# ViliamVadocz/takzero

Hardware: AMD Instinct MI355X
Metric: mcts_simulations_per_s (higher is better)
Workload: dtype f16

## Files before the change

bindings/takzero-hip-sys/src/lib.rs:

```rust
#![allow(non_camel_case_types, clippy::too_many_arguments)]
use std::os::raw::{c_char, c_int, c_uint, c_void};

pub const TZ_MAX_N: c_int = 6;
pub const TZ_MAX_SQUARES: c_int = 36;
pub const TZ_MAX_ACTIONS: c_int = 512;
pub const TZ_MAX_ACTIONS_6: c_int = 1024;
pub const TZ_OK: c_int = 0;
pub const TZ_EINVAL: c_int = -1;
pub const TZ_EPARSE: c_int = -2;
pub const TZ_EDEVICE: c_int = -3;
pub const TZ_ENOMEM: c_int = -4;
pub const TZ_ECAPACITY: c_int = -5;
pub const TZ_ESTATE: c_int = -6;
pub const TZ_ENUMERIC: c_int = -7;
pub const TZ_EMPTY: c_int = 0;
pub const TZ_FLAT: c_int = 1;
pub const TZ_WALL: c_int = 2;
pub const TZ_CAP: c_int = 3;
pub const TZ_EVAL_VALUE: c_int = 0;
pub const TZ_EVAL_WIN: c_int = 1;
pub const TZ_EVAL_LOSS: c_int = 2;
pub const TZ_EVAL_DRAW: c_int = 3;
pub const TZ_TERMINAL_NONE: c_int = -1;
pub const TZ_TERMINAL_WIN: c_int = 0;
// ... 168 lines not shown
    pub fn tz_reanalyze_take_text(ra: *mut TzReanalyze, out: *mut c_char, cap: u64, size_out: *mut u64) -> c_int;
    pub fn tz_reanalyze_run(ra: *mut TzReanalyze, directory: *const c_char, iterations: c_int, min_positions: c_int, suffix: *const c_char, reload: Option<unsafe extern "C" fn(*mut c_void) -> c_int>, reload_user: *mut c_void, wait_limit_s: f64) -> c_int;
    pub fn tz_compete(white: *mut TzSearch, black: *mut TzSearch, games: *const TzState, white_beta: f32, black_beta: f32, seed: u64, sampled_actions: c_int, search_budget: c_int, max_moves: c_int, result_out: *mut i32) -> c_int;
    pub fn tz_puzzle_benchmark(search: *mut TzSearch, puzzles: *const TzState, solutions: *const u16, count: c_int, win: c_int, seed: u64, sampled_actions: c_int, search_budget: c_int, result_out: *mut i32) -> c_int;
    pub fn tz_format_targets(n: c_int, count: c_int, states: *const TzState, moves: *const u16, policy: *const f32, nmoves: *const i32, amax: c_int, value: *const f32, ube: *const f32, out: *mut c_char, cap: u64, written_out: *mut u64) -> c_int;
    pub fn tz_parse_targets(text: *const c_char, len: u64, n: c_int, half_komi: c_int, max_targets: c_int, amax: c_int, states: *mut TzState, moves: *mut u16, policy: *mut f32, nmoves: *mut i32, value: *mut f32, ube: *mut f32, count_out: *mut i32, consumed_out: *mut u64, skipped_out: *mut i32) -> c_int;
    pub fn tz_trainer_create(board_n: c_int, arch: c_int, device_id: c_int, blocks: c_int, batch: c_int, learning_rate: f32, out: *mut *mut TzTrainer) -> c_int;
    pub fn tz_trainer_destroy(t: *mut TzTrainer) -> c_int;
    pub fn tz_trainer_tensor_count(t: *mut TzTrainer) -> c_int;
    pub fn tz_trainer_tensor_info(t: *mut TzTrainer, i: c_int, name_out: *mut c_char, name_cap: c_int, count_out: *mut u64) -> c_int;
    pub fn tz_trainer_set_tensor(t: *mut TzTrainer, name: *const c_char, what: c_int, data: *const f32, count: u64) -> c_int;
    pub fn tz_trainer_get_tensor(t: *mut TzTrainer, name: *const c_char, what: c_int, out: *mut f32, count: u64) -> c_int;
    pub fn tz_trainer_step(t: *mut TzTrainer, states: *const TzState, target_policy: *const f32, mask: *const u8, target_value: *const f32, target_ube: *const f32, train_ube: c_int, apply_step: c_int, losses_out: *mut f32) -> c_int;
    pub fn tz_trainer_outputs(t: *mut TzTrainer, policy_out: *mut f32, value_out: *mut f32, ube_out: *mut f32) -> c_int;
    pub fn tz_trainer_activation(t: *mut TzTrainer, layer: c_int, out: *mut f32, out_cap: u64) -> c_int;
    pub fn tz_trainer_shape(t: *mut TzTrainer, board_n_out: *mut c_int, batch_out: *mut c_int, arch_out: *mut c_int) -> c_int;
    pub fn tz_trainer_load(t: *mut TzTrainer, path: *const c_char) -> c_int;
    pub fn tz_trainer_save(t: *mut TzTrainer, path: *const c_char) -> c_int;
    pub fn tz_trainer_load_weights_mem(t: *mut TzTrainer, data: *const c_void, bytes: usize) -> c_int;
    pub fn tz_trainer_get_extras(t: *mut TzTrainer, out: *mut c_void, cap: u64, bytes_out: *mut u64) -> c_int;
    pub fn tz_trainer_from_net(t: *mut TzTrainer, net: *mut TzNet) -> c_int;
    pub fn tz_trainer_to_net(t: *mut TzTrainer, net: *mut TzNet) -> c_int;
    pub fn tz_learn_create(trainer: *mut TzTrainer, half_komi: c_int, seed: u64, selfplay_forced_uses: c_int, reanalyze_forced_uses: c_int, out: *mut *mut TzLearn) -> c_int;
    pub fn tz_learn_destroy(l: *mut TzLearn) -> c_int;
    pub fn tz_learn_feed(l: *mut TzLearn, which: c_int, path: *const c_char, model_steps: c_int, added_out: *mut u64) -> c_int;
    pub fn tz_learn_add_lines(l: *mut TzLearn, which: c_int, text: *const c_char, len: u64, model_steps: c_int, added_out: *mut u64) -> c_int;
    pub fn tz_learn_buffer_len(l: *mut TzLearn, which: c_int, len_out: *mut u64) -> c_int;
    pub fn tz_learn_step(l: *mut TzLearn, using_reanalyze: c_int, train_ube: c_int, augment: c_int, losses_out: *mut f32) -> c_int;
    pub fn tz_learn_last_batch(l: *mut TzLearn, states_out: *mut TzState, policy_out: *mut f32, mask_out: *mut u8, value_out: *mut f32, ube_out: *mut f32) -> c_int;
    pub fn tz_learn_run(l: *mut TzLearn, directory: *const c_char, starting_steps: i64, steps: i64, min_selfplay: c_int, min_reanalyze: c_int, steps_before_reanalyze: i64, read_interval_s: f64, sleep_s: f64, wait_limit_s: f64, on_step: Option<unsafe extern "C" fn(*mut c_void, i64, *const f32, *const TzState, c_int) -> c_int>, user: *mut c_void, model_steps_out: *mut i64) -> c_int;
    pub fn tz_learn_set_save_points(l: *mut TzLearn, steps_per_save: c_int, steps_per_checkpoint: c_int, hash_net: *mut TzNet) -> c_int;
    pub fn tz_device_math(op: c_int, a: *const f32, b: *const f32, out: *mut f32, n: c_int) -> c_int;
    pub fn tz_debug_conv_bench(net: *mut TzNet, variant: c_int, positions: c_int, iters: c_int, ms_out: *mut f32) -> c_int;
    pub fn tz_debug_tower_bench(net: *mut TzNet, variant: c_int, positions: c_int, iters: c_int, ms_out: *mut f32) -> c_int;
    pub fn tz_debug_net_clock(net: *mut TzNet, mhz_out: *mut f64, tower_us_out: *mut f64) -> c_int;
    pub fn tz_debug_net_stamps(net: *mut TzNet, out: *mut u64, max_groups: c_int, groups_out: *mut c_int) -> c_int;
}
```

include/takzero_hip.h:

```cpp
#ifndef TAKZERO_HIP_H
#define TAKZERO_HIP_H

#include <stddef.h>
#include <stdint.h>

#ifdef __cplusplus
extern "C" {
#endif

#define TZ_MAX_N 6
#define TZ_MAX_SQUARES 36
#define TZ_MAX_ACTIONS 512
#define TZ_MAX_ACTIONS_6 1024

#define TZ_OK 0
#define TZ_EINVAL (-1)
#define TZ_EPARSE (-2)
#define TZ_EDEVICE (-3)
#define TZ_ENOMEM (-4)
#define TZ_ECAPACITY (-5)
#define TZ_ESTATE (-6)
#define TZ_ENUMERIC (-7)

#define TZ_EMPTY 0
// ... 190 lines not shown
int tz_trainer_tensor_info(tz_trainer* t, int i, char* name_out, int name_cap, uint64_t* count_out);
int tz_trainer_set_tensor(tz_trainer* t, const char* name, int what, const float* data, uint64_t count);
int tz_trainer_get_tensor(tz_trainer* t, const char* name, int what, float* out, uint64_t count);
int tz_trainer_step(tz_trainer* t, const tz_state* states, const float* target_policy, const uint8_t* mask,
                    const float* target_value, const float* target_ube, int train_ube, int apply_step,
                    float* losses_out);
int tz_trainer_outputs(tz_trainer* t, float* policy_out, float* value_out, float* ube_out);
int tz_trainer_activation(tz_trainer* t, int layer, float* out, uint64_t out_cap);

int tz_trainer_shape(tz_trainer* t, int* board_n_out, int* batch_out, int* arch_out);
int tz_trainer_load(tz_trainer* t, const char* path);
int tz_trainer_save(tz_trainer* t, const char* path);
int tz_trainer_load_weights_mem(tz_trainer* t, const void* data, size_t bytes);
int tz_trainer_get_extras(tz_trainer* t, void* out, uint64_t cap, uint64_t* bytes_out);
int tz_trainer_from_net(tz_trainer* t, tz_net* net);
int tz_trainer_to_net(tz_trainer* t, tz_net* net);

typedef struct tz_learn tz_learn;
int tz_learn_create(tz_trainer* trainer, int half_komi, uint64_t seed, int selfplay_forced_uses, int reanalyze_forced_uses,
                    tz_learn** out);
int tz_learn_destroy(tz_learn* l);
int tz_learn_feed(tz_learn* l, int which, const char* path, int model_steps, uint64_t* added_out);
int tz_learn_add_lines(tz_learn* l, int which, const char* text, uint64_t len, int model_steps, uint64_t* added_out);
int tz_learn_buffer_len(tz_learn* l, int which, uint64_t* len_out);
int tz_learn_step(tz_learn* l, int using_reanalyze, int train_ube, int augment, float* losses_out);
int tz_learn_last_batch(tz_learn* l, tz_state* states_out, float* policy_out, uint8_t* mask_out, float* value_out, float* ube_out);
int tz_learn_run(tz_learn* l, const char* directory, int64_t starting_steps, int64_t steps, int min_selfplay, int min_reanalyze,
                 int64_t steps_before_reanalyze, double read_interval_s, double sleep_s, double wait_limit_s,
                 int (*on_step)(void*, int64_t, const float*, const tz_state*, int), void* user, int64_t* model_steps_out);
int tz_learn_set_save_points(tz_learn* l, int steps_per_save, int steps_per_checkpoint, tz_net* hash_net);

int tz_device_math(int op, const float* a, const float* b, float* out, int n);
int tz_debug_conv_bench(tz_net* net, int variant, int positions, int iters, float* ms_out);
int tz_debug_tower_bench(tz_net* net, int variant, int positions, int iters, float* ms_out);
int tz_debug_net_clock(tz_net* net, double* mhz_out, double* tower_us_out);
int tz_debug_net_stamps(tz_net* net, unsigned long long* out, int max_groups, int* groups_out);

#ifdef __cplusplus
}
#endif
#endif
```

takzero_amd/_lib.py:

```python
import ctypes as C
import os

import numpy as np

HERE = os.path.dirname(os.path.abspath(__file__))
LIB_PATH = os.path.join(HERE, "libtakzero_hip.so")
MAX_SQ = 36

STATE_DTYPE = np.dtype([
    ("colors", np.uint64, (MAX_SQ,)), ("height", np.uint8, (MAX_SQ,)), ("top", np.uint8, (MAX_SQ,)),
    ("stones", np.uint8, (2,)), ("caps", np.uint8, (2,)), ("to_move", np.uint8), ("n", np.uint8),
    ("half_komi", np.int8), ("pad0", np.uint8), ("ply", np.uint16), ("reversible_plies", np.uint16),
], align=True)
ROOT_INFO_DTYPE = np.dtype([
    ("visit_count", np.uint32), ("n_children", np.uint32), ("eval_tag", np.uint8),
    ("is_terminal_env", np.uint8), ("ply", np.uint16), ("eval_bits", np.uint32),
    ("std_dev", np.float32), ("logit", np.float32), ("probability", np.float32)], align=True)
assert STATE_DTYPE.itemsize == 376 and ROOT_INFO_DTYPE.itemsize == 28

SYMBOLS = [
    "tz_last_error", "tz_version", "tz_device_count", "tz_state_from_tps", "tz_state_to_tps", "tz_move_to_ptn",
    "tz_move_from_ptn", "tz_policy_size", "tz_input_channels", "tz_net_create", "tz_net_load_weights",
    "tz_net_load_weights_mem", "tz_net_destroy", "tz_net_eval", "tz_net_encode", "tz_net_forward_raw", "tz_net_hash_indices", "tz_net_load_bitset", "tz_net_save_bitset",
    "tz_search_create", "tz_search_destroy", "tz_search_set_positions", "tz_search_get_positions",
    "tz_search_new_openings", "tz_search_simulate", "tz_search_apply_noise", "tz_search_root_info",
    "tz_search_root_children", "tz_search_node", "tz_search_select_best_actions", "tz_search_improved_policy", "tz_search_ube_target",
    "tz_search_step", "tz_search_restart_terminal", "tz_search_gumbel_sh", "tz_search_counters", "tz_search_sync", "tz_search_pool_usage",
    "tz_search_profile", "tz_device_math", "tz_debug_conv_bench", "tz_debug_tower_bench", "tz_net_load_prepare", "tz_net_load_commit", "tz_net_load_discard", "tz_debug_net_clock", "tz_debug_net_stamps", "tz_search_terminal_details", "tz_search_play_moves",
    "tz_trainer_create", "tz_trainer_destroy", "tz_trainer_tensor_count", "tz_trainer_tensor_info",
    "tz_trainer_set_tensor", "tz_trainer_get_tensor", "tz_trainer_step", "tz_trainer_outputs", "tz_trainer_activation",
    "tz_format_targets", "tz_parse_targets", "tz_search_improved_policy_each", "tz_search_shape",
    "tz_selfplay_create", "tz_selfplay_destroy", "tz_selfplay_play_move", "tz_selfplay_counters", "tz_selfplay_take_text",
    "tz_selfplay_run", "tz_reanalyze_create", "tz_reanalyze_destroy", "tz_reanalyze_feed", "tz_reanalyze_iterate",
    "tz_reanalyze_take_text", "tz_reanalyze_run", "tz_compete", "tz_puzzle_benchmark", "tz_search_pool_overflows", "tz_trainer_shape",
    "tz_net_init_random", "tz_net_load_partial", "tz_net_save", "tz_net_clone", "tz_net_get_tensor", "tz_weights_convert", "tz_net_tensor_count", "tz_net_tensor_info",
    "tz_comm_unique_id", "tz_comm_rendezvous_id", "tz_comm_create_rccl", "tz_comm_create_fs", "tz_comm_destroy", "tz_comm_info",
    "tz_comm_all_gather", "tz_comm_take", "tz_comm_broadcast", "tz_comm_barrier", "tz_net_broadcast", "tz_selfplay_set_comm", "tz_selfplay_exchange",
    "tz_trainer_load", "tz_trainer_save", "tz_trainer_load_weights_mem", "tz_trainer_get_extras", "tz_trainer_from_net", "tz_trainer_to_net", "tz_learn_set_save_points",
    "tz_learn_create", "tz_learn_destroy", "tz_learn_feed", "tz_learn_add_lines", "tz_learn_buffer_len", "tz_learn_step", "tz_learn_run", "tz_learn_last_batch",
    "tz_search_simulate_batch", "tz_search_principal_variation", "tz_search_batch_profile",
    "tz_search_set_selection", "tz_search_get_selection",
]

_lib = None


class TakzeroError(RuntimeError):
    def __init__(self, code, msg):
        super().__init__("libtakzero_hip error %d: %s" % (code, msg))
        self.code = code


def load():
    global _lib
    if _lib is not None:
        return _lib
    if not os.path.exists(LIB_PATH):
        try:
            from . import build as _build

            _build.build()
# ... 48 lines not shown
    lib.tz_search_create.argtypes = [vp, ci, ci, ci, ci, ci, C.POINTER(vp)]
    lib.tz_search_destroy.argtypes = [vp]
    lib.tz_search_set_positions.argtypes = [vp, ci, vp, vp]
    lib.tz_search_get_positions.argtypes = [vp, vp]
    lib.tz_search_new_openings.argtypes = [vp, vp]
    lib.tz_search_simulate.argtypes = [vp, vp, ci]
    lib.tz_search_simulate_batch.argtypes = [vp, vp, ci, ci]
    lib.tz_search_batch_profile.argtypes = [vp] + [C.POINTER(C.c_double)] * 3 + [C.POINTER(C.c_uint64)]
    lib.tz_search_set_selection.argtypes = [vp, ci]
    lib.tz_search_get_selection.argtypes = [vp, C.POINTER(ci)]
    lib.tz_search_principal_variation.argtypes = [vp, ci, vp, ci, C.POINTER(ci)]
    lib.tz_search_apply_noise.argtypes = [vp, vp, ci, cf]
    lib.tz_search_root_info.argtypes = [vp, vp]
    lib.tz_search_root_children.argtypes = [vp, ci] + [vp] * 7
    lib.tz_search_node.argtypes = [vp, ci, vp, ci, vp, ci] + [vp] * 7
    lib.tz_search_select_best_actions.argtypes = [vp, vp]
    lib.tz_search_improved_policy.argtypes = [vp, cf, ci, vp]
    lib.tz_search_improved_policy_each.argtypes = [vp, vp, ci, vp]
    lib.tz_search_ube_target.argtypes = [vp, cf, vp]
    lib.tz_search_step.argtypes = [vp, vp]
    lib.tz_search_restart_terminal.argtypes = [vp, vp, vp]
    lib.tz_search_gumbel_sh.argtypes = [vp, vp, ci, ci, vp, ci, vp]
    lib.tz_search_counters.argtypes = [vp, C.POINTER(C.c_uint64), C.POINTER(C.c_uint64)]
    lib.tz_search_sync.argtypes = [vp]
    lib.tz_search_pool_overflows.argtypes = [vp, C.POINTER(C.c_uint64)]
    lib.tz_search_pool_usage.argtypes = [vp, C.POINTER(C.c_uint32), C.POINTER(C.c_uint32)]
    lib.tz_search_profile.argtypes = [vp, ci, C.POINTER(C.c_double), C.POINTER(C.c_uint64), C.POINTER(C.c_double),
                                      C.POINTER(C.c_uint64)]
    lib.tz_search_terminal_details.argtypes = [vp, vp, vp]
    lib.tz_search_play_moves.argtypes = [vp, vp, vp]
    lib.tz_device_math.argtypes = [ci, vp, vp, vp, ci]
    lib.tz_debug_conv_bench.argtypes = [vp, ci, ci, ci, C.POINTER(C.c_float)]
    lib.tz_debug_tower_bench.argtypes = [vp, ci, ci, ci, C.POINTER(C.c_float)]
    lib.tz_debug_net_clock.argtypes = [vp, C.POINTER(C.c_double), C.POINTER(C.c_double)]
    lib.tz_debug_net_stamps.argtypes = [vp, C.POINTER(C.c_uint64), C.c_int, C.POINTER(C.c_int)]
    lib.tz_net_load_prepare.argtypes = [vp, C.c_char_p, C.POINTER(vp)]
    lib.tz_net_load_commit.argtypes = [vp, vp]
    lib.tz_net_load_discard.argtypes = [vp]
    lib.tz_format_targets.argtypes = [ci, ci, vp, vp, vp, vp, ci, vp, vp, vp, C.c_uint64, C.POINTER(C.c_uint64)]
    lib.tz_parse_targets.argtypes = [vp, C.c_uint64, ci, ci, ci, ci, vp, vp, vp, vp, vp, vp, C.POINTER(C.c_int32),
                                     C.POINTER(C.c_uint64), C.POINTER(C.c_int32)]
    lib.tz_search_shape.argtypes = [vp] + [C.POINTER(ci)] * 4
    lib.tz_selfplay_create.argtypes = [vp, ci, C.c_uint64, ci, ci, ci, ci, C.POINTER(vp)]
    lib.tz_selfplay_destroy.argtypes = [vp]
    lib.tz_selfplay_play_move.argtypes = [vp]
    lib.tz_selfplay_counters.argtypes = [vp] + [C.POINTER(C.c_uint64)] * 3
    lib.tz_selfplay_take_text.argtypes = [vp, ci, vp, C.c_uint64, C.POINTER(C.c_uint64)]
    lib.tz_selfplay_run.argtypes = [vp, C.c_char_p, ci, ci, C.c_char_p, vp, vp, C.c_double]
    lib.tz_reanalyze_create.argtypes = [vp, ci, C.c_uint64, ci, ci, ci, ci, C.POINTER(vp)]
    lib.tz_reanalyze_destroy.argtypes = [vp]
    lib.tz_reanalyze_feed.argtypes = [vp, C.c_char_p, C.POINTER(C.c_uint64), C.POINTER(C.c_uint64)]
    lib.tz_reanalyze_iterate.argtypes = [vp]
    lib.tz_reanalyze_take_text.argtypes = [vp, vp, C.c_uint64, C.POINTER(C.c_uint64)]
    lib.tz_reanalyze_run.argtypes = [vp, C.c_char_p, ci, ci, C.c_char_p, vp, vp, C.c_double]
    lib.tz_compete.argtypes = [vp, vp, vp, cf, cf, C.c_uint64, ci, ci, ci, vp]
    lib.tz_puzzle_benchmark.argtypes = [vp, vp, vp, ci, ci, C.c_uint64, ci, ci, vp]
    lib.tz_trainer_shape.argtypes = [vp] + [C.POINTER(ci)] * 3
    lib.tz_learn_create.argtypes = [vp, ci, C.c_uint64, ci, ci, C.POINTER(vp)]
    lib.tz_learn_destroy.argtypes = [vp]
    lib.tz_learn_feed.argtypes = [vp, ci, C.c_char_p, ci, C.POINTER(C.c_uint64)]
    lib.tz_learn_add_lines.argtypes = [vp, ci, vp, C.c_uint64, ci, C.POINTER(C.c_uint64)]
    lib.tz_learn_buffer_len.argtypes = [vp, ci, C.POINTER(C.c_uint64)]
    lib.tz_learn_step.argtypes = [vp, ci, ci, ci, vp]
    lib.tz_learn_last_batch.argtypes = [vp, vp, vp, vp, vp, vp]
    lib.tz_learn_run.argtypes = [vp, C.c_char_p, C.c_int64, C.c_int64, ci, ci, C.c_int64, C.c_double, C.c_double, C.c_double, vp, vp,
                                 C.POINTER(C.c_int64)]
# ... 17 lines not shown
```

takzero_amd/csrc/tz_nn.hip:

```cpp
#include "tz_nn.h"
#include "tz_fp8.h"
#include "tz_fp6.h"
#include <type_traits>
#include "tz_ot.h"

#include <algorithm>
#include <cmath>
#include <cstdio>
#include <cstdlib>
#include <cstring>
#include <atomic>
#include <map>
#include <memory>
#include <mutex>
#include <thread>

int tz_nn_launch_split(int sp, int n, const void* net_args, int max_positions, hipStream_t st);
int tz_nn_launch_c6(int n, const void* net_args, int max_positions, hipStream_t st);
size_t tz_nn_c6_seed_bytes(int n, int max_positions);

namespace {

typedef float f32x4 __attribute__((ext_vector_type(4)));
typedef unsigned int u32x4 __attribute__((ext_vector_type(4)));
// ... 234 lines not shown
#pragma unroll
                for (int rt = 0; rt < RT; rt++) {
#pragma unroll
                    for (int j = 0; j < RN; j++)
                        acc[rt][j] = Elem<ET>::mfma(bq[kc & 3][j], av[rt], acc[rt][j]);
                    if constexpr ((ABL & 1) == 0) {
                        if (kc < 7) av[rt] = *reinterpret_cast<const ex8*>(lds + abase[rt] + (kc + 1 - (LAYOUT == 1 && kc >= 4 ? 4 : 0)) * KSTEP);
                        else av[rt] = *reinterpret_cast<const ex8*>(lds + abase[rt]);
                    }
                }
            }
        }
    } else {
        int yx[RT];
#pragma unroll
        for (int rt = 0; rt < RT; rt++) {
            const int r = rt * 16 + lr, px = r % NN;
            yx[rt] = r < ROWS ? ((px / NB) | ((px % NB) << 8)) : 0x7f7f;
        }
#pragma unroll
        for (int rt = 0; rt < RT; rt++)
#pragma unroll
            for (int j = 0; j < RN; j++) acc[rt][j] = f32x4{0.f, 0.f, 0.f, 0.f};
        const int nslices = (a.cin_pad + 255) / 256;
        constexpr int NLOAD = FROM_STATE ? 1 : (LROWS * 32 + NT - 1) / NT;
        uint4 stage[NLOAD];
        auto fetch_slice = [&](int slice) {
            const int cpr_s = min(256, a.cin_pad - slice * 256) / 8;
            const uint16_t* in = reinterpret_cast<const uint16_t*>(a.in) + (size_t)blockIdx.z * a.in_z + slice * 256;
#pragma unroll
            for (int i = 0; i < NLOAD; i++) {
                const int id = tid + i * NT, row = id >> 5, ci = id & 31;
                stage[i] = make_uint4(0, 0, 0, 0);
                if (row < valid_rows && ci < cpr_s) stage[i] = *reinterpret_cast<const uint4*>(in + (m0 + row) * a.in_stride + ci * 8);
            }
        };
        if constexpr (!FROM_STATE) fetch_slice(0);
        for (int slice = 0; slice < nslices; slice++) {
            const int cs = min(256, a.cin_pad - slice * 256);
            const int kcs = cs / 32, cpr = cs / 8;
            __syncthreads();
            if constexpr (FROM_STATE) {
                for (int row = tid; row < LROWS; row += NT) {
                    const bool ok = row < valid_rows;
                    const tz_state* s = nullptr;
                    int px = 0, fd = 0;
                    if (ok) {
                        const int pos = pos0 + row / NN;
                        px = row % NN;
                        s = a.states + (a.game_index ? a.game_index[pos] : pos);
                        fd = state_flat_diff<NB>(s);
                    }
                    for (int c8 = 0; c8 < cpr; c8++) {
                        ex8 v;
#pragma unroll
                        for (int k = 0; k < 8; k++) {
                            const int c = c8 * 8 + k;
                            v[k] = (ET)((ok && c < a.cin_real) ? plane_value<NB>(s, px, c, fd) : 0.0f);
                        }
                        *reinterpret_cast<ex8*>(lds + LdsImg<LAYOUT>::store_addr(row, c8, PLANE)) = v;
                    }
                }
            } else {
#pragma unroll
                for (int i = 0; i < NLOAD; i++) {
                    const int id = tid + i * NT, row = id >> 5, ci = id & 31;
                    if (row < LROWS && ci < cpr) *reinterpret_cast<uint4*>(lds + LdsImg<LAYOUT>::store_addr(row, ci, PLANE)) = stage[i];
                }
                if (slice + 1 < nslices) fetch_slice(slice + 1);
            }
            __syncthreads();
            ex8 bnext[RN];
#pragma unroll
            for (int j = 0; j < RN; j++) bnext[j] = wload(0, slice * 8, j);
            if constexpr (TAPS == 1) {
                int abase[RT];
                tap_bases<NB, RT, TAPS, LAYOUT>(yx, 0, lr, q, ZROW, abase);
                ex8 av[RT];
#pragma unroll
                for (int rt = 0; rt < RT; rt++) av[rt] = *reinterpret_cast<const ex8*>(lds + abase[rt]);
                for (int kc = 0; kc < kcs; kc++) {
                    ex8 bcur[RN];
#pragma unroll
                    for (int j = 0; j < RN; j++) bcur[j] = bnext[j];
                    if (kc + 1 < kcs) {
#pragma unroll
                        for (int j = 0; j < RN; j++) bnext[j] = wload(0, slice * 8 + kc + 1, j);
                    }
                    __builtin_amdgcn_sched_barrier(0);
#pragma unroll
                    for (int rt = 0; rt < RT; rt++) {
#pragma unroll
                        for (int j = 0; j < RN; j++) acc[rt][j] = Elem<ET>::mfma(bcur[j], av[rt], acc[rt][j]);
                        if (kc + 1 < kcs) av[rt] = *reinterpret_cast<const ex8*>(lds + abase[rt] + (kc + 1) * KSTEP);
                    }
                }
                continue;
            }
            for (int tap = 0; tap < TAPS; tap++) {
                int abase[RT];
                tap_bases<NB, RT, TAPS, LAYOUT>(yx, tap, lr, q, ZROW, abase);
                for (int kc = 0; kc < kcs; kc++) {
                    ex8 bcur[RN];
#pragma unroll
                    for (int j = 0; j < RN; j++) bcur[j] = bnext[j];
                    if (kc + 1 < kcs) {
#pragma unroll
                        for (int j = 0; j < RN; j++) bnext[j] = wload(tap, slice * 8 + kc + 1, j);
                    } else if (tap + 1 < TAPS) {
#pragma unroll
                        for (int j = 0; j < RN; j++) bnext[j] = wload(tap + 1, slice * 8, j);
                    }
#pragma unroll
                    for (int rt = 0; rt < RT; rt++) {
                        const ex8 av = *reinterpret_cast<const ex8*>(lds + abase[rt] + kc * KSTEP);
#pragma unroll
                        for (int j = 0; j < RN; j++)
                            acc[rt][j] = Elem<ET>::mfma(bcur[j], av, acc[rt][j]);
                    }
                }
            }
        }
    }

#pragma unroll
    for (int j = 0; j < RN; j++) {
        const int cbase = (ct0 + j) * 16 + q * 4;
        const f32x4 bias = *reinterpret_cast<const f32x4*>(a.bias + (size_t)blockIdx.z * a.bias_z + cbase);
#pragma unroll
        for (int rt = 0; rt < RT; rt++) {
            const int r = rt * 16 + lr;
            if (r >= valid_rows) continue;
            f32x4 v = acc[rt][j] + bias;
            const size_t o = (size_t)blockIdx.z * a.out_z + (m0 + r) * a.out_stride + cbase;
            if (a.has_res) {
                const ex4 rv = *reinterpret_cast<const ex4*>(reinterpret_cast<const uint16_t*>(a.residual) + o);
#pragma unroll
                for (int k = 0; k < 4; k++) v[k] += (float)rv[k];
            }
            if (a.relu) {
#pragma unroll
                for (int k = 0; k < 4; k++) v[k] = v[k] > 0.f ? v[k] : 0.f;
            }
            if (a.out_f32) {
                *reinterpret_cast<f32x4*>(reinterpret_cast<float*>(a.out) + o) = v;
            } else {
                ex4 ov;
#pragma unroll
                for (int k = 0; k < 4; k++) ov[k] = Elem<ET>::cvt(v[k]);
                *reinterpret_cast<ex4*>(reinterpret_cast<uint16_t*>(a.out) + o) = ov;
            }
        }
    }
}

struct TowerArgs {
    const uint16_t* in;
    uint16_t* out;
    const uint16_t* w;
    const float* bias;
    const int32_t* count_dev;
    int count_host;
    int nlayers;
};

template <int NB, int P, int OPT = 0, typename ET = __bf16>
__global__ __launch_bounds__(512, 2) void tower_mfma_kernel(TowerArgs a) {
    typedef typename Elem<ET>::x8 ex8;
    typedef typename Elem<ET>::x4 ex4;
    constexpr int RN = 2, TAPS = 9, LAYOUT = 1, NT = 512;
    constexpr int NN = NB * NB, ROWS = P * NN, RT = (ROWS + 15) / 16, LROWS = RT * 16 + 8, ZROW = RT * 16;
    constexpr int PLANE = LROWS * LDS_ROWB, KSTEP = PLANE;
// ... 2487 lines not shown
}

__host__ __device__ constexpr int ppt_small(int nb) { return nb == 1 ? 64 : nb == 3 ? 7 : nb == 4 ? 6 : nb == 5 ? 4 : 3; }

int conv_cfg() {
    static int cfg = -1;
    if (cfg < 0) {
        const char* e = getenv("TZ_CONV_CFG");
        cfg = e ? atoi(e) : 0;
    }
    return cfg;
}

template <int NB, int P, int NW, int RN, int TAPS, bool FROM_STATE, bool SINGLE, int ABL = 0, int LAYOUT = 1, typename ET = __bf16, int OCC = 2>
int launch_conv(const ConvArgs& a, int max_positions, int n_blocks_y, hipStream_t st) {
    constexpr int NN = NB * NB, RT = (P * NN + 15) / 16, LROWS = RT * 16 + 8;
    const size_t smem = LdsImg<LAYOUT>::bytes(LROWS);
    auto kern = conv_mfma_kernel<NB, P, RN, TAPS, FROM_STATE, ABL, SINGLE, NW, LAYOUT, ET, OCC>;
    static bool attr_done[64] = {};
    int attr_dev = 0;
    TZ_HIP(hipGetDevice(&attr_dev));
    bool& attr_set = attr_done[attr_dev & 63];
    if (!attr_set) {
        TZ_HIP(hipFuncSetAttribute(reinterpret_cast<const void*>(kern), hipFuncAttributeMaxDynamicSharedMemorySize, (int)smem));
        attr_set = true;
    }
    dim3 grid((max_positions + P - 1) / P, n_blocks_y, a.groups > 1 ? a.groups : 1);
    hipLaunchKernelGGL(kern, grid, dim3(NW * 64), smem, st, a);
    hipError_t e = hipGetLastError();
    if (e != hipSuccess) return tz_fail(TZ_EDEVICE, std::string("conv launch: ") + hipGetErrorString(e));
    return TZ_OK;
}

int linear_grouped_bf16(int precision, const uint16_t* w, const float* bias, int groups, int cin_pad, int cout_pad, const void* in,
                        int in_stride, int in_z, void* out, int out_stride, int out_z, bool relu, bool out_f32,
                        const int32_t* count_dev, int count_host, int max_positions, hipStream_t st) {
    ConvArgs a;
    memset(&a, 0, sizeof a);
    a.in = in;
    a.count_dev = count_dev;
    a.count_host = count_host;
    a.w = w;
    a.bias = bias;
    a.out = out;
    a.cin_pad = cin_pad;
    a.kc_total = cin_pad / 32;
    a.ct_total = cout_pad / 16;
    a.out_stride = out_stride;
    a.cin_real = cin_pad;
    a.relu = relu;
    a.out_f32 = out_f32;
    a.in_stride = in_stride;
    a.groups = groups;
    a.in_z = in_z;
    a.w_z_frags = a.kc_total * a.ct_total;
    a.bias_z = cout_pad;
    a.out_z = out_z;
    if (max_positions <= 128) {
        if (prec_is_f16(precision)) return launch_conv<1, 32, 8, 2, 1, false, false, 0, 1, _Float16>(a, max_positions, cout_pad / 256, st);
        return launch_conv<1, 32, 8, 2, 1, false, false>(a, max_positions, cout_pad / 256, st);
    }
    if (prec_is_f16(precision)) return launch_conv<1, 128, 8, 2, 1, false, false, 0, 1, _Float16>(a, max_positions, cout_pad / 256, st);
    return launch_conv<1, 128, 8, 2, 1, false, false>(a, max_positions, cout_pad / 256, st);
}

template <int NB, typename ET>
int conv_board(const ConvArgs& a, int cout_pad, bool from_state, int max_positions, hipStream_t st) {
    constexpr int PA = ppt_for(NB), PB = ppt_small(NB);
    const bool wide = cout_pad % 256 == 0;
    const int by = wide ? cout_pad / 256 : cout_pad / 128;
    if (conv_cfg() == 0) {
        if (from_state) return launch_conv<NB, PA, 8, 2, 9, true, false, 0, 1, ET>(a, max_positions, by, st);
        if (wide) return launch_conv<NB, PA, 8, 2, 9, false, true, 0, 1, ET>(a, max_positions, by, st);
        return launch_conv<NB, PA, 8, 1, 9, false, true, 0, 1, ET>(a, max_positions, by, st);
    }
    if (from_state) return launch_conv<NB, PB, 4, 4, 9, true, false, 0, 1, ET>(a, max_positions, by, st);
    if (wide) return launch_conv<NB, PB, 4, 4, 9, false, true, 0, 1, ET>(a, max_positions, by, st);
    return launch_conv<NB, PB, 4, 2, 9, false, true, 0, 1, ET>(a, max_positions, by, st);
}

template <typename ET>
int conv_dispatch(int n, bool board, const ConvArgs& a, int cout_pad, bool from_state, int max_positions, hipStream_t st) {
    if (!board) return launch_conv<1, 64, 8, 2, 1, false, false, 0, 1, ET>(a, max_positions, cout_pad / 256, st);
    switch (n) {
        case 3: return conv_board<3, ET>(a, cout_pad, from_state, max_positions, st);
        case 4: return conv_board<4, ET>(a, cout_pad, from_state, max_positions, st);
        case 5: return conv_board<5, ET>(a, cout_pad, from_state, max_positions, st);
        case 6: return conv_board<6, ET>(a, cout_pad, from_state, max_positions, st);
    }
    return tz_fail(TZ_EINVAL, "conv: unsupported board size");
}

int conv_bf16(tz_net* net, const ConvW& L, const void* in, const tz_state* states, const int32_t* gidx,
              const int32_t* count_dev, int count_host, int max_positions, const void* residual, void* out,
              int out_stride, bool relu, bool out_f32, bool board, hipStream_t st) {
    ConvArgs a;
// ... 1051 lines not shown
                case 0: rc = launch_conv<5, ppt_for(5), 8, 2, 9, false, true, 0>(a, positions, 1, net->stream); break;
#ifdef TZ_ABLATIONS
                case 1: rc = launch_conv<5, ppt_for(5), 8, 2, 9, false, true, 1>(a, positions, 1, net->stream); break;
                case 2: rc = launch_conv<5, ppt_for(5), 8, 2, 9, false, true, 2>(a, positions, 1, net->stream); break;
                case 3: rc = launch_conv<5, ppt_for(5), 8, 2, 9, false, true, 3>(a, positions, 1, net->stream); break;
                case 4: rc = launch_conv<5, ppt_for(5), 8, 2, 1, false, true, 0>(a, positions, 1, net->stream); break;
                case 20: rc = launch_conv<5, ppt_for(5), 8, 2, 9, false, true, 0, 0>(a, positions, 1, net->stream); break;
                case 21: rc = launch_conv<5, ppt_for(5), 8, 2, 9, false, true, 1, 0>(a, positions, 1, net->stream); break;
                case 23: rc = launch_conv<5, ppt_for(5), 8, 2, 9, false, true, 3, 0>(a, positions, 1, net->stream); break;
                case 30: rc = launch_conv<5, ppt_for(5), 4, 4, 9, false, true, 0, 1, __bf16, 1>(a, positions, 1, net->stream); break;
                case 31: rc = launch_conv<5, ppt_for(5), 4, 4, 9, false, true, 1, 1, __bf16, 1>(a, positions, 1, net->stream); break;
                case 33: rc = launch_conv<5, ppt_for(5), 4, 4, 9, false, true, 3, 1, __bf16, 1>(a, positions, 1, net->stream); break;
                case 10: rc = launch_conv<5, ppt_small(5), 4, 4, 9, false, true, 0>(a, positions, 1, net->stream); break;
                case 11: rc = launch_conv<5, ppt_small(5), 4, 4, 9, false, true, 1>(a, positions, 1, net->stream); break;
                case 12: rc = launch_conv<5, ppt_small(5), 4, 4, 9, false, true, 2>(a, positions, 1, net->stream); break;
                case 13: rc = launch_conv<5, ppt_small(5), 4, 4, 9, false, true, 3>(a, positions, 1, net->stream); break;
                case 14: rc = launch_conv<5, ppt_small(5), 4, 4, 1, false, true, 0>(a, positions, 1, net->stream); break;
#endif
                default: rc = tz_fail(TZ_EINVAL, "tz_debug_conv_bench: unknown variant (the ablation variants need a build with --ablations)");
            }
        }
        return rc;
    };
    if ((rc = run(3))) return rc;
    TZ_HIP(hipEventRecord(e0, net->stream));
    if ((rc = run(iters))) return rc;
    TZ_HIP(hipEventRecord(e1, net->stream));
    TZ_HIP(hipEventSynchronize(e1));
    float ms = 0.f;
    TZ_HIP(hipEventElapsedTime(&ms, e0, e1));
    (void)hipEventDestroy(e0);
    (void)hipEventDestroy(e1);
    *ms_out = ms / iters;
    return TZ_OK;
}

int tz_debug_tower_bench(tz_net* net, int variant, int positions, int iters, float* ms_out) {
    if (!net || !net->loaded || net->n != 5 || net->precision != TZ_PREC_BF16 || !net->tower_w)
        return tz_fail(TZ_EINVAL, "tz_debug_tower_bench: needs a loaded 5x5 bf16 network");
    TZ_HIP(hipSetDevice(net->device));
    int rc = tz_net_ensure_batch(net, positions);
    if (rc) return rc;
    {
        std::vector<uint16_t> h((size_t)positions * 25 * FILTERS);
        uint32_t x = 999u;
        for (auto& v : h) {
            x = x * 1664525u + 1013904223u;
            v = (x >> 31) ? 0 : f2bf((float)((x >> 8) % 10001) * 1e-4f);
        }
        TZ_HIP(hipMemcpy(net->act_a, h.data(), h.size() * 2, hipMemcpyHostToDevice));
    }
    TowerArgs a;
    a.in = reinterpret_cast<const uint16_t*>(net->act_a);
    a.out = reinterpret_cast<uint16_t*>(net->act_b);
    a.w = net->tower_w;
    a.bias = net->tower_bias;
    a.count_dev = nullptr;
    a.count_host = positions;
    a.nlayers = 2 * net->blocks;
    hipEvent_t e0, e1;
    TZ_HIP(hipEventCreate(&e0));
    TZ_HIP(hipEventCreate(&e1));
    auto run = [&](int n) -> int {
        int r = TZ_OK;
        for (int i = 0; i < n && !r; i++) {
            switch (variant) {
// ... 346 lines not shown
```

Baseline: 1.498 million.

## Add dedicated pipelined MFMA linear kernel for RND MLP layers with adaptive tile size

Adds a linear_mfma_kernel for the large-batch RND linear layers. It double-buffers 256-channel activation slices in LDS through buffer loads, prefetches weight fragments two k-steps ahead, and replaces the generic conv kernel for batches above 128 positions. The tile is 64 positions when the 128-position grid would leave CUs idle, otherwise 128. The aim is to hide global and LDS latency behind MFMA work and to fill the GPU better on small grids, at the cost of another kernel and more template instantiations. It also adds debug benchmark and buffer-readback entry points and ablation hooks in the conv kernel.

```diff
diff --git a/bindings/takzero-hip-sys/src/lib.rs b/bindings/takzero-hip-sys/src/lib.rs
--- a/bindings/takzero-hip-sys/src/lib.rs
+++ b/bindings/takzero-hip-sys/src/lib.rs
@@ -224,6 +224,8 @@
     pub fn tz_learn_set_save_points(l: *mut TzLearn, steps_per_save: c_int, steps_per_checkpoint: c_int, hash_net: *mut TzNet) -> c_int;
     pub fn tz_device_math(op: c_int, a: *const f32, b: *const f32, out: *mut f32, n: c_int) -> c_int;
     pub fn tz_debug_conv_bench(net: *mut TzNet, variant: c_int, positions: c_int, iters: c_int, ms_out: *mut f32) -> c_int;
+    pub fn tz_debug_linear_bench(net: *mut TzNet, variant: c_int, layer: c_int, positions: c_int, iters: c_int, ms_out: *mut f32) -> c_int;
+    pub fn tz_debug_rnd_buffer(net: *mut TzNet, which: c_int, out: *mut c_void, bytes: usize) -> c_int;
     pub fn tz_debug_tower_bench(net: *mut TzNet, variant: c_int, positions: c_int, iters: c_int, ms_out: *mut f32) -> c_int;
     pub fn tz_debug_net_clock(net: *mut TzNet, mhz_out: *mut f64, tower_us_out: *mut f64) -> c_int;
     pub fn tz_debug_net_stamps(net: *mut TzNet, out: *mut u64, max_groups: c_int, groups_out: *mut c_int) -> c_int;
diff --git a/include/takzero_hip.h b/include/takzero_hip.h
--- a/include/takzero_hip.h
+++ b/include/takzero_hip.h
@@ -246,6 +246,8 @@
 
 int tz_device_math(int op, const float* a, const float* b, float* out, int n);
 int tz_debug_conv_bench(tz_net* net, int variant, int positions, int iters, float* ms_out);
+int tz_debug_linear_bench(tz_net* net, int variant, int layer, int positions, int iters, float* ms_out);
+int tz_debug_rnd_buffer(tz_net* net, int which, void* out, size_t bytes);
 int tz_debug_tower_bench(tz_net* net, int variant, int positions, int iters, float* ms_out);
 int tz_debug_net_clock(tz_net* net, double* mhz_out, double* tower_us_out);
 int tz_debug_net_stamps(tz_net* net, unsigned long long* out, int max_groups, int* groups_out);
diff --git a/takzero_amd/_lib.py b/takzero_amd/_lib.py
--- a/takzero_amd/_lib.py
+++ b/takzero_amd/_lib.py
@@ -26,7 +26,7 @@
     "tz_search_new_openings", "tz_search_simulate", "tz_search_apply_noise", "tz_search_root_info",
     "tz_search_root_children", "tz_search_node", "tz_search_select_best_actions", "tz_search_improved_policy", "tz_search_ube_target",
     "tz_search_step", "tz_search_restart_terminal", "tz_search_gumbel_sh", "tz_search_counters", "tz_search_sync", "tz_search_pool_usage",
-    "tz_search_profile", "tz_device_math", "tz_debug_conv_bench", "tz_debug_tower_bench", "tz_net_load_prepare", "tz_net_load_commit", "tz_net_load_discard", "tz_debug_net_clock", "tz_debug_net_stamps", "tz_search_terminal_details", "tz_search_play_moves",
+    "tz_search_profile", "tz_device_math", "tz_debug_conv_bench", "tz_debug_tower_bench", "tz_debug_linear_bench", "tz_debug_rnd_buffer", "tz_net_load_prepare", "tz_net_load_commit", "tz_net_load_discard", "tz_debug_net_clock", "tz_debug_net_stamps", "tz_search_terminal_details", "tz_search_play_moves",
     "tz_trainer_create", "tz_trainer_destroy", "tz_trainer_tensor_count", "tz_trainer_tensor_info",
     "tz_trainer_set_tensor", "tz_trainer_get_tensor", "tz_trainer_step", "tz_trainer_outputs", "tz_trainer_activation",
     "tz_format_targets", "tz_parse_targets", "tz_search_improved_policy_each", "tz_search_shape",
@@ -141,6 +141,8 @@
     lib.tz_device_math.argtypes = [ci, vp, vp, vp, ci]
     lib.tz_debug_conv_bench.argtypes = [vp, ci, ci, ci, C.POINTER(C.c_float)]
     lib.tz_debug_tower_bench.argtypes = [vp, ci, ci, ci, C.POINTER(C.c_float)]
+    lib.tz_debug_linear_bench.argtypes = [vp, ci, ci, ci, ci, C.POINTER(C.c_float)]
+    lib.tz_debug_rnd_buffer.argtypes = [vp, ci, vp, C.c_size_t]
     lib.tz_debug_net_clock.argtypes = [vp, C.POINTER(C.c_double), C.POINTER(C.c_double)]
     lib.tz_debug_net_stamps.argtypes = [vp, C.POINTER(C.c_uint64), C.c_int, C.POINTER(C.c_int)]
     lib.tz_net_load_prepare.argtypes = [vp, C.c_char_p, C.POINTER(vp)]
diff --git a/takzero_amd/csrc/tz_nn.hip b/takzero_amd/csrc/tz_nn.hip
--- a/takzero_amd/csrc/tz_nn.hip
+++ b/takzero_amd/csrc/tz_nn.hip
@@ -290,6 +290,10 @@
             for (int i = 0; i < NLOAD; i++) {
                 const int id = tid + i * NT, row = id >> 5, ci = id & 31;
                 stage[i] = make_uint4(0, 0, 0, 0);
+                if constexpr ((ABL & 4) != 0) {
+                    stage[i] = make_uint4(0x38003c00u + row, 0x3a003400u, 0x3c003800u + ci, 0x34003a00u);
+                    continue;
+                }
                 if (row < valid_rows && ci < cpr_s) stage[i] = *reinterpret_cast<const uint4*>(in + (m0 + row) * a.in_stride + ci * 8);
             }
         };
@@ -319,7 +323,7 @@
                         *reinterpret_cast<ex8*>(lds + LdsImg<LAYOUT>::store_addr(row, c8, PLANE)) = v;
                     }
                 }
-            } else {
+            } else if ((ABL & 4) == 0 || slice == 0) {
 #pragma unroll
                 for (int i = 0; i < NLOAD; i++) {
                     const int id = tid + i * NT, row = id >> 5, ci = id & 31;
@@ -341,7 +345,7 @@
                     ex8 bcur[RN];
 #pragma unroll
                     for (int j = 0; j < RN; j++) bcur[j] = bnext[j];
-                    if (kc + 1 < kcs) {
+                    if ((ABL & 2) == 0 && kc + 1 < kcs) {
 #pragma unroll
                         for (int j = 0; j < RN; j++) bnext[j] = wload(0, slice * 8 + kc + 1, j);
                     }
@@ -350,7 +354,7 @@
                     for (int rt = 0; rt < RT; rt++) {
 #pragma unroll
                         for (int j = 0; j < RN; j++) acc[rt][j] = Elem<ET>::mfma(bcur[j], av[rt], acc[rt][j]);
-                        if (kc + 1 < kcs) av[rt] = *reinterpret_cast<const ex8*>(lds + abase[rt] + (kc + 1) * KSTEP);
+                        if ((ABL & 1) == 0 && kc + 1 < kcs) av[rt] = *reinterpret_cast<const ex8*>(lds + abase[rt] + (kc + 1) * KSTEP);
                     }
                 }
                 continue;
@@ -396,6 +400,151 @@
 #pragma unroll
                 for (int k = 0; k < 4; k++) v[k] += (float)rv[k];
             }
+            if (a.relu) {
+#pragma unroll
+                for (int k = 0; k < 4; k++) v[k] = v[k] > 0.f ? v[k] : 0.f;
+            }
+            if (a.out_f32) {
+                *reinterpret_cast<f32x4*>(reinterpret_cast<float*>(a.out) + o) = v;
+            } else {
+                ex4 ov;
+#pragma unroll
+                for (int k = 0; k < 4; k++) ov[k] = Elem<ET>::cvt(v[k]);
+                *reinterpret_cast<ex4*>(reinterpret_cast<uint16_t*>(a.out) + o) = ov;
+            }
+        }
+    }
+}
+
+template <int P, typename ET = __bf16, int ABL = 0>
+__global__ __launch_bounds__(512, 2) void linear_mfma_kernel(ConvArgs a) {
+    typedef typename Elem<ET>::x8 ex8;
+    typedef typename Elem<ET>::x4 ex4;
+    constexpr int NT = 512, NW = 8, RN = 2, RT = P / 16;
+    constexpr int PLANE = P * LDS_ROWB + 64, IMG = 8 * PLANE;
+    constexpr int NLOAD = P * 32 / NT;
+    static_assert(P % 16 == 0 && (P * 32) % NT == 0 && NLOAD <= 8, "a slice is stored within its 8 k-steps");
+    static_assert((RT - 1) * 16 * LDS_ROWB + 7 * PLANE < 65536, "fragment reads are one base register + immediates");
+    extern __shared__ __attribute__((aligned(16))) unsigned char lds[];
+    const int count = a.count_dev ? *a.count_dev : a.count_host;
+    const int pos0 = blockIdx.x * P;
+    if (pos0 >= count) return;
+    const int tid = threadIdx.x, lane = tid & 63;
+    const int wave = __builtin_amdgcn_readfirstlane(tid >> 6);
+    const int q = lane >> 4, lr = lane & 15;
+    const int valid_rows = min(P, count - pos0);
+    const size_t m0 = (size_t)pos0;
+    const int ct0 = (blockIdx.y * NW + wave) * RN;
+    const __amdgpu_buffer_rsrc_t wrsrc = __builtin_amdgcn_make_buffer_rsrc(
+        const_cast<uint16_t*>(a.w), 0, (a.groups > 1 ? a.groups * a.w_z_frags : a.kc_total * a.ct_total) * 1024, 0x00020000);
+    const int lane16 = lane * 16;
+    const int kc_total = a.kc_total;
+    auto wload = [&](int kcg, int j) -> ex8 {
+        const int frag = (int)blockIdx.z * a.w_z_frags + kcg * a.ct_total + (ct0 + j);
+        const u32x4 r = __builtin_amdgcn_raw_buffer_load_b128(wrsrc, lane16, frag * 1024, 0);
+        return __builtin_bit_cast(ex8, r);
+    };
+    const int nslices = (a.cin_pad + 255) / 256;
+    const int srow = tid >> 5, sci = tid & 31;
+    const int pitch = a.in_stride * 2;
+    const __amdgpu_buffer_rsrc_t arsrc = __builtin_amdgcn_make_buffer_rsrc(
+        const_cast<uint16_t*>(reinterpret_cast<const uint16_t*>(a.in) + (size_t)blockIdx.z * a.in_z + m0 * a.in_stride), 0,
+        (valid_rows - 1) * pitch + a.cin_pad * 2, 0x00020000);
+    const int voff0 = srow * pitch + sci * 16;
+    uint4 stage[NLOAD];
+    auto fetch_piece = [&](int slice_off, int i) {
+        if constexpr ((ABL & 4) == 0) {
+            const u32x4 r = __builtin_amdgcn_raw_buffer_load_b128(arsrc, voff0 + i * 16 * pitch + slice_off, 0, 0);
+            stage[i] = __builtin_bit_cast(uint4, r);
+        } else {
+            stage[i] = make_uint4(0x38003c00u + srow, 0x3a003400u, 0x3c003800u + sci, 0x34003a00u);
+        }
+    };
+    constexpr int NO_SLICE = 0x40000000;
+    const int sbase = LdsImg<1>::store_addr(srow, sci, PLANE);
+    const int abase = LdsImg<1>::read_base(true, lr, q, 0);
+
+#pragma unroll
+    for (int i = 0; i < NLOAD; i++) fetch_piece(0, i);
+    ex8 bq[4][RN];
+#pragma unroll
+    for (int j = 0; j < RN; j++) {
+        bq[0][j] = wload(0, j);
+        bq[1][j] = wload(min(1, kc_total - 1), j);
+    }
+    f32x4 acc[RT][RN];
+#pragma unroll
+    for (int rt = 0; rt < RT; rt++)
+#pragma unroll
+        for (int j = 0; j < RN; j++) acc[rt][j] = f32x4{0.f, 0.f, 0.f, 0.f};
+#pragma unroll
+    for (int i = 0; i < NLOAD; i++) *reinterpret_cast<uint4*>(lds + sbase + i * 16 * LDS_ROWB) = stage[i];
+    {
+        const int off = nslices > 1 ? 512 : NO_SLICE;
+#pragma unroll
+        for (int i = 0; i < NLOAD; i++) fetch_piece(off, i);
+    }
+    __syncthreads();
+
+    ex8 av[RT];
+    auto k_step = [&](auto store, int kc, int g, const unsigned char* img, unsigned char* other, int next2_off) {
+        constexpr bool STORE = decltype(store)::value;
+        if constexpr ((ABL & 2) == 0) {
+#pragma unroll
+            for (int j = 0; j < RN; j++) bq[(kc + 2) & 3][j] = wload(min(g + 2, kc_total - 1), j);
+        }
+        if constexpr (STORE && (ABL & 4) == 0) {
+            if (kc < NLOAD) {
+                *reinterpret_cast<uint4*>(other + kc * 16 * LDS_ROWB) = stage[kc];
+                fetch_piece(next2_off, kc);
+            }
+        }
+        __builtin_amdgcn_sched_barrier(0);
+#pragma unroll
+        for (int rt = 0; rt < RT; rt++) {
+#pragma unroll
+            for (int j = 0; j < RN; j++) acc[rt][j] = Elem<ET>::mfma(bq[kc & 3][j], av[rt], acc[rt][j]);
+            if constexpr ((ABL & 1) == 0) {
+                if (kc < 7) av[rt] = *reinterpret_cast<const ex8*>(img + rt * 16 * LDS_ROWB + (kc + 1) * PLANE);
+            }
+        }
+    };
+    int slice = 0;
+    for (; slice + 1 < nslices; slice++) {
+        const unsigned char* img = lds + (slice & 1) * IMG + abase;
+        unsigned char* other = lds + ((slice & 1) ^ 1) * IMG + sbase;
+        const int next2_off = slice + 2 < nslices ? (slice + 2) * 512 : NO_SLICE;
+#pragma unroll
+        for (int rt = 0; rt < RT; rt++) av[rt] = *reinterpret_cast<const ex8*>(img + rt * 16 * LDS_ROWB);
+#pragma unroll
+        for (int kc = 0; kc < 8; kc++) k_step(std::true_type{}, kc, slice * 8 + kc, img, other, next2_off);
+        __syncthreads();
+    }
+    {
+        const unsigned char* img = lds + (slice & 1) * IMG + abase;
+        const int kcs = kc_total - slice * 8;
+#pragma unroll
+        for (int rt = 0; rt < RT; rt++) av[rt] = *reinterpret_cast<const ex8*>(img + rt * 16 * LDS_ROWB);
+        if (kcs == 8) {
+#pragma unroll
+            for (int kc = 0; kc < 8; kc++) k_step(std::false_type{}, kc, slice * 8 + kc, img, nullptr, 0);
+        } else {
+#pragma unroll
+            for (int kc = 0; kc < 7; kc++)
+                if (kc < kcs) k_step(std::false_type{}, kc, slice * 8 + kc, img, nullptr, 0);
+        }
+    }
+
+#pragma unroll
+    for (int j = 0; j < RN; j++) {
+        const int cbase = (ct0 + j) * 16 + q * 4;
+        const f32x4 bias = *reinterpret_cast<const f32x4*>(a.bias + (size_t)blockIdx.z * a.bias_z + cbase);
+#pragma unroll
+        for (int rt = 0; rt < RT; rt++) {
+            const int r = rt * 16 + lr;
+            if (r >= valid_rows) continue;
+            f32x4 v = acc[rt][j] + bias;
+            const size_t o = (size_t)blockIdx.z * a.out_z + (m0 + r) * a.out_stride + cbase;
             if (a.relu) {
 #pragma unroll
                 for (int k = 0; k < 4; k++) v[k] = v[k] > 0.f ? v[k] : 0.f;
@@ -2949,6 +3098,43 @@
     return TZ_OK;
 }
 
+template <int P, typename ET, int ABL = 0>
+int launch_linear(const ConvArgs& a, int max_positions, int n_blocks_y, hipStream_t st) {
+    constexpr size_t smem = 2 * 8 * ((size_t)P * LDS_ROWB + 64);
+    auto kern = linear_mfma_kernel<P, ET, ABL>;
+    static bool attr_done[64] = {};
+    int attr_dev = 0;
+    TZ_HIP(hipGetDevice(&attr_dev));
+    bool& attr_set = attr_done[attr_dev & 63];
+    if (!attr_set) {
+        TZ_HIP(hipFuncSetAttribute(reinterpret_cast<const void*>(kern), hipFuncAttributeMaxDynamicSharedMemorySize, (int)smem));
+        attr_set = true;
+    }
+    dim3 grid((max_positions + P - 1) / P, n_blocks_y, a.groups > 1 ? a.groups : 1);
+    hipLaunchKernelGGL(kern, grid, dim3(512), smem, st, a);
+    hipError_t e = hipGetLastError();
+    if (e != hipSuccess) return tz_fail(TZ_EDEVICE, std::string("linear launch: ") + hipGetErrorString(e));
+    return TZ_OK;
+}
+
+int rnd_gemm_cfg() {
+    static int cfg = -1;
+    if (cfg < 0) {
+        const char* e = getenv("TZ_RND_GEMM");
+        cfg = !e ? 0 : !strcmp(e, "conv") ? 1 : !strcmp(e, "p128") ? 128 : !strcmp(e, "p64") ? 64 : 0;
+    }
+    return cfg;
+}
+
+int device_cu_count() {
+    static int cus[64] = {};
+    int dev = 0;
+    if (hipGetDevice(&dev) != hipSuccess) return 256;
+    int& c = cus[dev & 63];
+    if (c == 0 && hipDeviceGetAttribute(&c, hipDeviceAttributeMultiprocessorCount, dev) != hipSuccess) c = 256;
+    return c;
+}
+
 int linear_grouped_bf16(int precision, const uint16_t* w, const float* bias, int groups, int cin_pad, int cout_pad, const void* in,
                         int in_stride, int in_z, void* out, int out_stride, int out_z, bool relu, bool out_f32,
                         const int32_t* count_dev, int count_host, int max_positions, hipStream_t st) {
@@ -2977,8 +3163,18 @@
         if (prec_is_f16(precision)) return launch_conv<1, 32, 8, 2, 1, false, false, 0, 1, _Float16>(a, max_positions, cout_pad / 256, st);
         return launch_conv<1, 32, 8, 2, 1, false, false>(a, max_positions, cout_pad / 256, st);
     }
-    if (prec_is_f16(precision)) return launch_conv<1, 128, 8, 2, 1, false, false, 0, 1, _Float16>(a, max_positions, cout_pad / 256, st);
-    return launch_conv<1, 128, 8, 2, 1, false, false>(a, max_positions, cout_pad / 256, st);
+    const int cfg = rnd_gemm_cfg();
+    if (cfg == 1) {
+        if (prec_is_f16(precision)) return launch_conv<1, 128, 8, 2, 1, false, false, 0, 1, _Float16>(a, max_positions, cout_pad / 256, st);
+        return launch_conv<1, 128, 8, 2, 1, false, false>(a, max_positions, cout_pad / 256, st);
+    }
+    const bool half_tiles = cfg ? cfg == 64 : (max_positions + 127) / 128 * (cout_pad / 256) * groups < device_cu_count();
+    if (half_tiles) {
+        if (prec_is_f16(precision)) return launch_linear<64, _Float16>(a, max_positions, cout_pad / 256, st);
+        return launch_linear<64, __bf16>(a, max_positions, cout_pad / 256, st);
+    }
+    if (prec_is_f16(precision)) return launch_linear<128, _Float16>(a, max_positions, cout_pad / 256, st);
+    return launch_linear<128, __bf16>(a, max_positions, cout_pad / 256, st);
 }
 
 template <int NB, typename ET>
@@ -4096,6 +4292,102 @@
     (void)hipEventDestroy(e0);
     (void)hipEventDestroy(e1);
     *ms_out = ms / iters;
+    return TZ_OK;
+}
+
+int tz_debug_linear_bench(tz_net* net, int variant, int layer, int positions, int iters, float* ms_out) {
+    if (!net || !net->loaded || !net->has_rnd || net->n != 5 || net->precision == TZ_PREC_F32 || layer < 0 || layer > 2 || positions <= 128 || iters < 1)
+        return tz_fail(TZ_EINVAL, "tz_debug_linear_bench: needs a loaded 5x5 net5 in a 16-bit precision, layer 0..2 and more than 128 positions");
+    TZ_HIP(hipSetDevice(net->device));
+    int rc = tz_net_ensure_batch(net, positions);
+    if (rc) return rc;
+    const int in_pad = (net->cin * net->nn + 31) / 32 * 32;
+    const bool f16 = prec_is_f16(net->precision);
+    {
+        std::vector<uint16_t> h((size_t)positions * 2048);
+        uint32_t x = 4242u;
+        for (auto& v : h) {
+            x = x * 1664525u + 1013904223u;
+            const float f = ((int)(x >> 8) % 20001 - 10000) * 1e-4f;
+            v = f16 ? f2h(f) : f2bf(f);
+        }
+        TZ_HIP(hipMemcpy(net->rnd_in, h.data(), (size_t)positions * in_pad * 2, hipMemcpyHostToDevice));
+        TZ_HIP(hipMemcpy(net->rnd_h1, h.data(), h.size() * 2, hipMemcpyHostToDevice));
+        TZ_HIP(hipMemcpy(net->rnd_h2, h.data(), h.size() * 2, hipMemcpyHostToDevice));
+    }
+    ConvArgs a;
+    memset(&a, 0, sizeof a);
+    const int groups = layer == 0 ? 1 : 2, cin_pad = layer == 0 ? in_pad : 1024, cout_pad = layer == 0 ? 2048 : layer == 1 ? 1024 : 512;
+    a.in = layer == 0 ? net->rnd_in : layer == 1 ? net->rnd_h1 : net->rnd_h2;
+    a.out = layer == 0 ? net->rnd_h1 : layer == 1 ? net->rnd_h2 : (void*)net->rnd_out;
+    a.count_host = positions;
+    a.w = net->rndw[layer];
+    a.bias = net->rndb[layer];
+    a.cin_pad = a.cin_real = cin_pad;
+    a.kc_total = cin_pad / 32;
+    a.ct_total = cout_pad / 16;
+    a.out_stride = layer == 2 ? 1024 : 2048;
+    a.relu = layer != 2;
+    a.out_f32 = layer == 2;
+    a.in_stride = layer == 0 ? in_pad : 2048;
+    a.groups = groups;
+    a.in_z = layer == 0 ? 0 : 1024;
+    a.w_z_frags = a.kc_total * a.ct_total;
+    a.bias_z = cout_pad;
+    a.out_z = layer == 0 ? 0 : layer == 1 ? 1024 : 512;
+    const int by = cout_pad / 256;
+    auto one = [&](auto et) -> int {
+        typedef std::remove_pointer_t<decltype(et)> ET;
+        switch (variant) {
+            case 0: return launch_conv<1, 128, 8, 2, 1, false, false, 0, 1, ET>(a, positions, by, net->stream);
+            case 10: return launch_linear<128, ET>(a, positions, by, net->stream);
+            case 20: return launch_linear<64, ET>(a, positions, by, net->stream);
+#ifdef TZ_ABLATIONS
+            case 1: return launch_conv<1, 128, 8, 2, 1, false, false, 1, 1, ET>(a, positions, by, net->stream);
+            case 2: return launch_conv<1, 128, 8, 2, 1, false, false, 2, 1, ET>(a, positions, by, net->stream);
+            case 3: return launch_conv<1, 128, 8, 2, 1, false, false, 3, 1, ET>(a, positions, by, net->stream);
+            case 7: return launch_conv<1, 128, 8, 2, 1, false, false, 7, 1, ET>(a, positions, by, net->stream);
+            case 11: return launch_linear<128, ET, 1>(a, positions, by, net->stream);
+            case 12: return launch_linear<128, ET, 2>(a, positions, by, net->stream);
+            case 13: return launch_linear<128, ET, 3>(a, positions, by, net->stream);
+            case 17: return launch_linear<128, ET, 7>(a, positions, by, net->stream);
+            case 21: return launch_linear<64, ET, 1>(a, positions, by, net->stream);
+            case 22: return launch_linear<64, ET, 2>(a, positions, by, net->stream);
+            case 23: return launch_linear<64, ET, 3>(a, positions, by, net->stream);
+            case 27: return launch_linear<64, ET, 7>(a, positions, by, net->stream);
+#endif
+        }
+        return tz_fail(TZ_EINVAL, "tz_debug_linear_bench: unknown variant (the ablation variants need a build with --ablations)");
+    };
+    auto run = [&](int n) -> int {
+        int r = TZ_OK;
+        for (int i = 0; i < n && !r; i++) r = f16 ? one((_Float16*)nullptr) : one((__bf16*)nullptr);
+        return r;
+    };
+    hipEvent_t e0, e1;
+    TZ_HIP(hipEventCreate(&e0));
+    TZ_HIP(hipEventCreate(&e1));
+    if ((rc = run(3))) return rc;
+    TZ_HIP(hipEventRecord(e0, net->stream));
+    if ((rc = run(iters))) return rc;
+    TZ_HIP(hipEventRecord(e1, net->stream));
+    TZ_HIP(hipEventSynchronize(e1));
+    float ms = 0.f;
+    TZ_HIP(hipEventElapsedTime(&ms, e0, e1));
+    (void)hipEventDestroy(e0);
+    (void)hipEventDestroy(e1);
+    *ms_out = ms / iters;
+    return TZ_OK;
+}
+
+int tz_debug_rnd_buffer(tz_net* net, int which, void* out, size_t bytes) {
+    if (!net || !net->has_rnd || net->precision == TZ_PREC_F32 || which < 1 || which > 3 || !out)
+        return tz_fail(TZ_EINVAL, "tz_debug_rnd_buffer: needs a net5 in a 16-bit precision and which = 1..3");
+    const size_t have = which == 3 ? (size_t)2 * net->max_batch * 512 * sizeof(float) : (size_t)net->max_batch * 2048 * 2;
+    if (bytes > have) return tz_fail(TZ_EINVAL, "tz_debug_rnd_buffer: more bytes than the buffer holds");
+    TZ_HIP(hipSetDevice(net->device));
+    TZ_HIP(hipStreamSynchronize(net->stream));
+    TZ_HIP(hipMemcpy(out, which == 1 ? net->rnd_h1 : which == 2 ? net->rnd_h2 : (void*)net->rnd_out, bytes, hipMemcpyDeviceToHost));
     return TZ_OK;
 }
 
```

Result: no change. 1.508 million (median of 6 runs) (+0.6%).
